# HanzhiC/TexPose

Hardware: AMD Instinct MI355X
Metric: rendered rays/sec (480x640x128 samples) + train iters/sec (higher is better)
Workload: dtype f32 carried as 2xf16 (f16x3 products, f32 accumulate); 1 GPU; Duck-like synthetic scene 480x640, 128 samples/ray, batch=1 image per GPU, forward render (render_by_slices mode='val', all pixels), per-sample outputs materialised; samples_per_ray=128, mlp_precision=f16x3, parallelism=images sharded across 1 GPU(s), no collective

## Files before the change

include/texpose_amd.h:

```cpp
#ifndef TEXPOSE_AMD_H
#define TEXPOSE_AMD_H

#include <stddef.h>
#include <stdint.h>

#ifdef __cplusplus
extern "C" {
#endif

typedef void* tp_stream_t;

#define TP_ABI_VERSION 16

int tp_abi_version(void);
const char* tp_last_error(void);

enum tp_pixel_mode {
  TP_PIX_COORDS = 0,
  TP_PIX_INDEX = 1
};
enum tp_bounds_mode {
  TP_BOUNDS_MAP = 0,
  TP_BOUNDS_AABB = 1,
  TP_BOUNDS_NONE = 2
// ... 96 lines not shown
  unsigned int* act_max;
  float* ray_bias;
  const float* density_noise;
} tp_mlp_fwd_args;
size_t tp_mlp_ray_bias_bytes(int B, int R);
enum { TP_MLP_FP32 = 0, TP_MLP_F16X3 = 1, TP_MLP_F16 = 2 };

int tp_mlp_fwd(const tp_mlp_fwd_args* args, tp_stream_t stream);

size_t tp_mlp_packed_t_bytes(void);
size_t tp_mlp_bwd_workspace_bytes(int64_t n_samples);
typedef struct tp_mlp_bwd_args {
  tp_mlp_weights weights;
  void* packed_t;
  int repack;
  const float* saved;
  const float* rgb; const float* density; const float* uncert;
  const float* g_rgb; const float* g_density; const float* g_uncert;
  const float* lat_trans;
  const float* lat_light;
  int B, R, N;
  float* g_rgb_w[4];   float* g_rgb_b[4];
  float* g_trans_w[4]; float* g_trans_b[4];
  float* g_lat_trans;
  float* g_lat_light;
  void* workspace;
  int wgrad_precision;
  int dz_max_is_clear;
  int wgrad_cus;
} tp_mlp_bwd_args;
int tp_mlp_bwd(const tp_mlp_bwd_args* args, tp_stream_t stream);

int tp_posenc(const float* x, int64_t n, int C, int L, float* out, tp_stream_t stream);

typedef struct tp_composite_args {
  const float* ray;
  const float* rgb;
  const float* density;
  const float* depth;
  const float* uncert;
  int64_t n; int N; float min_uncert;
  float* out_ray;
  float* alpha_static;
  float* alpha_transient;
  float* prob;
  float* rgb_ray;
  float* uncert_ray;
} tp_composite_args;
int tp_composite_fwd(const tp_composite_args* args, tp_stream_t stream);

typedef struct tp_composite_bwd_args {
  tp_composite_args fwd;
  const float* g_out_ray;
  const float* g_alpha_static;
  const float* g_alpha_transient;
  const float* g_prob;
  float* g_rgb;
  float* g_density;
  float* g_uncert;
  const float* g_rgb_ray;
  const float* g_uncert_ray;
  const float* g_rgb_ray2;
  const float* g_rgb_ray3;
  const float* g_density_add;
} tp_composite_bwd_args;
int tp_composite_bwd(const tp_composite_bwd_args* args, tp_stream_t stream);

typedef struct tp_render_eval_args {
  tp_raygen_args raygen;
  const void* packed;
  const float* lat_trans;
  const float* lat_light;
  int precision;
  int* status;
  float min_uncert;
  void* workspace;
  float* out_ray;
  float* alpha_static;
  float* alpha_transient;
  int packed_ray_bias;
} tp_render_eval_args;
size_t tp_render_eval_workspace_bytes(int B, int R, int N);
int tp_render_eval(const tp_render_eval_args* args, tp_stream_t stream);

typedef struct tp_patch_gather_args {
  const float* coords;
  const float* image;
  const float* image_syn;
  const float* nocs;
  const float* normal;
  const float* obj_mask;
  const float* mask_syn;
  int B, P, H, W;
  float* out;
  const float* disc_rgb; float* disc_real; float* disc_fake; int disc_geo; int pad_;
} tp_patch_gather_args;
int tp_patch_gather(const tp_patch_gather_args* args, tp_stream_t stream);

typedef struct tp_eval_metrics_args {
  const float* rgb_static;
  const float* image;
  const float* obj_mask;
  int B, h, w;
  int out_h, out_w;
  void* workspace;
  double* out;
} tp_eval_metrics_args;
int64_t tp_eval_metrics_workspace_bytes(int B, int out_h, int out_w);
int tp_eval_metrics(const tp_eval_metrics_args* args, tp_stream_t stream);

#define TP_SN_MAX_WEIGHTS 8
#define TP_SN_MAX_SLABS 8
#define TP_SN_MAX_SETS 3
typedef struct tp_sn_weight {
  const float* weight;
  float* u;
  float* v;
  float* weight_sn;
  float* sigma;
  const float* grad_sn;
  float* grad;
  float* work;
  int rows, cols;
  float* u_out;
  float* v_out;
  int32_t accumulate;
  const float* grad_sn2; const float* weight_sn2; const float* u2; const float* v2; const float* sigma2;
} tp_sn_weight;
int64_t tp_sn_work_floats(int rows, int cols);
int tp_sn_fwd(const tp_sn_weight* weights, int n, int training, tp_stream_t stream);
int tp_sn_fwd_sets(const tp_sn_weight* weights, int n, int n_sets, tp_stream_t stream);
int tp_sn_bwd(const tp_sn_weight* weights, int n, tp_stream_t stream);
typedef struct tp_sn_step_tail {
  const float* terms[4]; float weights[4]; int n_terms; int word_finite;
  float* total;
  int32_t* bad; int32_t* snapshot; int n_bad; int pad_;
  float* param[TP_SN_MAX_WEIGHTS];
  float* square_avg[TP_SN_MAX_WEIGHTS];
  float* step[TP_SN_MAX_WEIGHTS];
  const float* lr_dev; float lr_host, alpha, one_minus_alpha, eps;
} tp_sn_step_tail;
int tp_sn_bwd_step(const tp_sn_weight* weights, int n, const tp_sn_step_tail* tail, tp_stream_t stream);

#define TP_NERF_LOSSES_MAX_BLOCKS 1024
typedef struct tp_nerf_losses_args {
  const float* rgb;
  const float* uncert;
  const float* density;
  const float* gathered;
  int B, P, N;
  void* workspace;
  double* sums;
  float* losses;
  uint32_t* ticket;
} tp_nerf_losses_args;
int tp_nerf_losses_fwd(const tp_nerf_losses_args* args, tp_stream_t stream);
int tp_nerf_losses_bwd(const tp_nerf_losses_args* args, const float* g_render, const float* g_unc, const float* g_trans,
                       float* g_rgb, float* g_uncert, float* g_density, tp_stream_t stream);
int tp_nerf_losses_bwd_total(const tp_nerf_losses_args* args, const float* g_render, const float* g_unc, const float* g_trans,
                             float* g_rgb, float* g_uncert, float* g_density, const float* const* terms, const float* weights, int n,
                             float* out, const int32_t* mlp_status, int32_t* bad, int n_bad, int word_status, int word_finite,
                             int32_t* snapshot, uint64_t* step_counter, tp_stream_t stream);

int tp_inorm_lrelu_fwd(const float* x, int64_t n_inst, int hw, float eps, float slope, float* y, float* xhat, float* rstd,
                       tp_stream_t stream);
int tp_inorm_lrelu_bwd(const float* xhat, const float* rstd, const float* gy, int64_t n_inst, int hw, float slope,
// ... 542 lines not shown
```

texpose_amd/csrc/render_eval.hip:

```cpp
#include "tp_common.h"

namespace {
size_t align256(size_t x) { return (x + 255) / 256 * 256; }
struct Layout { size_t center, ray, depth, rgb, density, uncert, mlp_ws, ray_bias, total; };
Layout layout(int64_t B, int64_t R, int64_t N) {
  Layout l;
  size_t o = 0;
  l.center = o; o += align256((size_t)B * R * 3 * 4);
  l.ray = o;    o += align256((size_t)B * R * 3 * 4);
  l.depth = o;  o += align256((size_t)B * R * N * 4);
  l.rgb = o;    o += align256((size_t)B * R * N * 6 * 4);
  l.density = o; o += align256((size_t)B * R * N * 2 * 4);
  l.uncert = o; o += align256((size_t)B * R * N * 4);
  l.mlp_ws = o; o += align256(tp_mlp_workspace_bytes(B * R * N));
  l.ray_bias = o; o += align256(tp_mlp_ray_bias_bytes((int)B, (int)R));
  l.total = o;
  return l;
}
}

extern "C" size_t tp_render_eval_workspace_bytes(int B, int R, int N) { return layout(B, R, N).total; }

extern "C" int tp_render_eval(const tp_render_eval_args* a, tp_stream_t stream) {
  TP_REQUIRE(a && a->workspace && a->out_ray && a->packed && a->lat_trans && a->lat_light, "null pointer");
  TP_REQUIRE(a->raygen.B > 0 && a->raygen.R > 0 && a->raygen.N > 0, "bad sizes");
  const int B = a->raygen.B, R = a->raygen.R, N = a->raygen.N;
  const Layout l = layout(B, R, N);
  char* ws = (char*)a->workspace;
  tp_raygen_args rg = a->raygen;
  rg.center = (float*)(ws + l.center); rg.ray = (float*)(ws + l.ray); rg.depth = (float*)(ws + l.depth);
  rg.near = nullptr; rg.far = nullptr;
  if (int rc = tp_raygen(&rg, stream)) return rc;
  tp_mlp_fwd_args m = {};
  m.packed = a->packed;
  m.center = rg.center; m.ray = rg.ray; m.depth = rg.depth;
  m.lat_trans = a->lat_trans; m.lat_light = a->lat_light;
  m.B = B; m.R = R; m.N = N;
  m.rgb = (float*)(ws + l.rgb); m.density = (float*)(ws + l.density); m.uncert = (float*)(ws + l.uncert);
  m.saved = nullptr; m.workspace = ws + l.mlp_ws; m.precision = a->precision; m.status = a->status;
  if (a->packed_ray_bias) {
    TP_REQUIRE((a->precision == TP_MLP_F16X3 || a->precision == TP_MLP_F16) && N % 128 == 0,
               "tp_render_eval: packed_ray_bias needs TP_MLP_F16X3 or TP_MLP_F16 and N % 128 == 0");
    m.ray_bias = (float*)(ws + l.ray_bias);
  }
  if (int rc = tp_mlp_fwd(&m, stream)) return rc;
  tp_composite_args c = {};
  c.ray = rg.ray; c.rgb = m.rgb; c.density = m.density; c.depth = rg.depth; c.uncert = m.uncert;
  c.n = (int64_t)B * R; c.N = N; c.min_uncert = a->min_uncert;
  c.out_ray = a->out_ray; c.alpha_static = a->alpha_static; c.alpha_transient = a->alpha_transient; c.prob = nullptr;
  return tp_composite_fwd(&c, stream);
}
```

texpose_amd/graph.py:

```python
from __future__ import annotations

import itertools
import warnings

import torch
import torch.nn.functional as torch_F

from . import autograd_ops, knobs, ops
from .geometry import FlexPatchSampler, RaySampler, rotation_distance
from .nerf import NeRF
from .options import AttrDict as edict

RENDER_KEYS = ("rgb", "rgb_static", "rgb_transient", "opacity", "opacity_static", "opacity_transient", "uncert",
               "depth", "alpha_static", "alpha_transient", "density")

_philox_calls = itertools.count()
_ones_cache = {}


def _ones_like_cached(t):
    key = (tuple(t.shape), t.dtype, str(t.device))
    if key not in _ones_cache:
        _ones_cache[key] = torch.ones_like(t).detach()
    return _ones_cache[key]


class RenderMixin:

    HOST_REQUIRED = ("nerf", "lab_loss", "latent_vars_trans", "latent_vars_light", "MSE_loss", "compute_gan_loss")
    HOST_OPTIONAL = (
        "fuse_prologue",
        "step_counter",
        "range_fallbacks",
        "perceptual_loss",
        "feat_stream",
    )

    @staticmethod
    def _jitter(opt, rand, step_counter=None):
        if rand is not None:
            return dict(rand=rand)
        if opt.nerf.sample_stratified and step_counter is not None:
            return dict(jitter=ops.JITTER_PHILOX, seed=torch.initial_seed() & (2 ** 64 - 1), offset=0, offset_dev=step_counter)
        if opt.nerf.sample_stratified:
            return dict(jitter=ops.JITTER_PHILOX, seed=torch.initial_seed() & (2 ** 64 - 1), offset=next(_philox_calls))
        return dict(jitter=ops.JITTER_MID)

    @staticmethod
    def sample_depth(opt, batch_size, depth_range, num_rays=None, rand=None):
        near, far = depth_range
        return ops.sample_depth(near, far, opt.nerf.sample_intvs, depth_param=RenderMixin._depth_param(opt), **RenderMixin._jitter(opt, rand))[..., None]

    @staticmethod
    def _depth_param(opt):
        param = opt.nerf.depth.param
        if param not in ops.DEPTH_PARAMS:
            raise KeyError(param)
        return param

    @staticmethod
    def ray_batch_sample(ray_identity, ray_idx):
        assert ray_identity.shape[0] == ray_idx.shape[0]
        C = ray_identity.shape[-1]
        return torch.gather(ray_identity, 1, ray_idx[..., None].expand(-1, -1, C))

    def render(self, opt, pose, intr=None, ray_idx=None, depth_range=None, sample_idx=None, mode=None, rand=None):
        N = opt.nerf.sample_intvs
        z_near, z_far = depth_range
        batch_size = len(pose)
        src = dict(coords=ray_idx) if mode == "train" else dict(ray_idx=ray_idx)
        rows_k13 = (mode == "train" and torch.is_tensor(sample_idx) and sample_idx.dim() == 1 and sample_idx.is_cuda
                    and self.latent_vars_trans.weight.shape[0] == self.latent_vars_light.weight.shape[0])
        fused = {}
        if mode == "train" and getattr(self, "fuse_prologue", False):
            job = ray_idx.__dict__.pop("_tp_sampler_job", None)
            if job is not None:
                fused["sampler"] = job
            if rows_k13:
                lat_t, lat_l, fused["rows"] = autograd_ops.latent_rows(self.latent_vars_trans.weight, self.latent_vars_light.weight, sample_idx,
                                                                       defer=True)
        elif torch.is_tensor(ray_idx) and "_tp_sampler_job" in ray_idx.__dict__:
            raise RuntimeError("render: ray_idx comes from a deferred sampler call but this render does not fill it (fuse_prologue is off)")
        center, ray, _, _, depth = ops.raygen(intr, pose, H=opt.H, W=opt.W, n_samples=N, z_near=z_near, z_far=z_far,
                                              ndc=bool(opt.camera.ndc), depth_param=self._depth_param(opt), **src, **fused,
                                              **self._jitter(opt, rand, getattr(self, "step_counter", None) if mode == "train" else None))
        depth_samples = depth[..., None]
        if "rows" in fused:
            pass
        elif rows_k13:
            lat_t, lat_l = autograd_ops.latent_rows(self.latent_vars_trans.weight, self.latent_vars_light.weight, sample_idx)
        elif mode == "train" and torch.is_tensor(sample_idx) and sample_idx.dim() == 1:
            lat_t = self.latent_vars_trans.weight.index_select(0, sample_idx)
            lat_l = self.latent_vars_light.weight.index_select(0, sample_idx)
        elif mode == "train":
            lat_t = self.latent_vars_trans.weight[sample_idx]
            lat_l = self.latent_vars_light.weight[sample_idx]
        elif mode == "val":
            lat_t = self.latent_vars_trans.weight[0][None]
            lat_l = self.latent_vars_light.weight[0][None]
        else:
            if opt.render.transient == "zero":
                lat_t = torch.zeros(batch_size, opt.nerf.N_latent_trans, device=pose.device)
            elif opt.render.transient == "sample":
                lat_t = self.latent_vars_trans.weight[sample_idx][None]
            else:
                raise NotImplementedError
            lat_l = self.latent_vars_light.weight[sample_idx][None]
        rgb_s, density_s, uncert_s = self.nerf.forward_samples(opt, center=center, ray=ray, depth_samples=depth_samples,
                                                               latent_variable_trans=lat_t, latent_variable_light=lat_l,
                                                               mode=mode)
        per_sample = bool(opt.render.get("per_sample", True)) or torch.is_grad_enabled()
        fan = dict(fan_out={}) if mode == "train" else {}
        (rgb, rgb_static, rgb_transient, depth_map, opacity, opacity_static, opacity_transient, _prob, uncert,
         alpha_static, alpha_transient) = self.nerf.composite(opt, ray, rgb_s, density_s, depth_samples, uncert_s,
                                                              per_sample=per_sample, want_prob=False, **fan)
        ret = edict(rgb=rgb, rgb_static=rgb_static, rgb_transient=rgb_transient, opacity=opacity,
                    opacity_static=opacity_static, opacity_transient=opacity_transient, uncert=uncert,
                    depth=depth_map, alpha_static=alpha_static, alpha_transient=alpha_transient, density=density_s)
        ret.update(fan.get("fan_out") or {})
        return ret

    def _range_guarded(self, opt, device, render_image):
        out = render_image()
        nerf = self.nerf
        if not set(ops.F16_RANGE_PRECISIONS) & {nerf.precision, nerf.train_precision} or opt.arch.get("mlp_range_check", "sync") == "off" \
                or torch.cuda.is_current_stream_capturing():
            return out
        if ops.take_mlp_status(device) & 1:
            self.range_fallbacks = getattr(self, "range_fallbacks", 0) + 1
            if self.range_fallbacks == 1:
                warnings.warn("texpose_amd: an activation left the fp16 range of the f16x3 / f16 MLP kernel; the image was "
                              "re-rendered with the exact-fp32 kernel (arch.mlp_precision='fp32' avoids the double work)")
            keep = nerf.precision, nerf.train_precision
            nerf.precision = nerf.train_precision = "fp32"
            try:
                out = render_image()
            finally:
                nerf.precision, nerf.train_precision = keep
        return out

    @staticmethod
    def _slice_rays(opt):
        return int(opt.nerf.get("slice_rays") or max(opt.nerf.rand_rays, min(opt.H * opt.W, 1 << 20)))

    def render_by_slices(self, opt, pose, intr=None, depth_range=None, object_mask=None, sample_idx=None, mode=None):
        return self._range_guarded(opt, pose.device, lambda: self._render_by_slices(
            opt, pose, intr=intr, depth_range=depth_range, object_mask=object_mask, sample_idx=sample_idx, mode=mode))

    def _render_by_slices(self, opt, pose, intr=None, depth_range=None, object_mask=None, sample_idx=None, mode=None):
        HW = opt.H * opt.W
        step = self._slice_rays(opt)
        if mode == "val":
            parts = {k: [] for k in RENDER_KEYS}
            for c in range(0, HW, step):
                idx = torch.arange(c, min(c + step, HW), device=pose.device)[None]
                ret = self.render(opt, pose, intr=intr, ray_idx=idx, depth_range=depth_range, sample_idx=sample_idx,
                                  mode=mode)
                for k in RENDER_KEYS:
                    parts[k].append(ret[k])
            return edict({k: (None if v[0] is None else (v[0] if len(v) == 1 else torch.cat(v, dim=1))) for k, v in parts.items()})
        dev, N = pose.device, opt.nerf.sample_intvs
        obj = (object_mask.reshape(HW) > 0).nonzero(as_tuple=True)[0]
        out = edict()
        lazy = not bool(opt.render.get("per_sample", True))
        for k in RENDER_KEYS:
            if lazy and "alpha" in k:
                out[k] = None
            elif k == "uncert":
                out[k] = torch.full((1, HW, 1), float(opt.nerf.min_uncert), device=dev)
            elif k == "density":
                out[k] = torch.ones(1, HW, N, 2, device=dev)
            elif "rgb" in k:
                out[k] = torch.zeros(1, HW, 3, device=dev)
            elif "alpha" in k:
                out[k] = torch.ones(1, HW, N, device=dev)
            else:
                out[k] = torch.zeros(1, HW, 1, device=dev)
        for c in range(0, len(obj), step):
            idx = obj[c:c + step][None]
            ret = self.render(opt, pose, intr=intr, ray_idx=idx, depth_range=depth_range, sample_idx=sample_idx,
                              mode=mode)
            for k in RENDER_KEYS:
                if out[k] is not None:
                    out[k][:, idx[0]] = ret[k][0]
        return out

    def gather_patches(self, opt, var, disc_rgb=None):
        B = len(var.idx)
        if var.get("gathered_for") is var.ray_idx:
            return var
        args = (var.ray_idx, var.image, var.get("image_syn", var.image),
                var.get("nocs_pred", var.image), var.get("normal_pred", var.image),
                var.obj_mask.view(B, opt.H, opt.W), var.get("mask_syn", var.obj_mask).view(B, opt.H, opt.W))
        if disc_rgb is not None and disc_rgb.is_cuda and not knobs.K.no_gather_disc:
            g, real, fake = ops.patch_gather(*args, disc_rgb=disc_rgb, disc_geo=bool(opt.gan.geo_conditional))
            var.disc_stacks = (real, fake, disc_rgb)
        else:
            g = ops.patch_gather(*args)
        var.gathered, var.gathered_for = g, var.ray_idx
        var.image_sample, var.image_syn_sample = g[:, 0:3], g[:, 3:6]
        var.nocs_sample, var.normal_sample = g[:, 6:9], g[:, 9:12]
        var.mask_sample, var.mask_syn_sample = g[:, 12:13], g[:, 13:14]
        return var

    def sample_geometry(self, opt, var, mode=None):
        if mode == "train":
            if "nocs_sample" not in var:
                var = self.gather_patches(opt, var)
            return var
        B = len(var.idx)
        ms = (var.mask_syn > 0).float().view(B, 1, opt.H, opt.W)
        var.nocs_sample, var.normal_sample = var.nocs_pred * ms, var.normal_pred * ms
        return var

    def evaluate_metrics(self, opt, var, lpips_module=None):
        out_hw = None if list(opt.data.image_size) == [128, 128] else (480, 640)
        psnr, ssim, _ = ops.eval_metrics(var.rgb_static, var.image, var.obj_mask, opt.H, opt.W, out_hw=out_hw)
        out = edict(psnr=psnr, ssim=ssim)
        if lpips_module is not None:
            B = var.image.shape[0]
            rgb_map = var.rgb_static.view(B, opt.H, opt.W, 3).permute(0, 3, 1, 2)
            image, mask = var.image.view(B, 3, opt.H, opt.W), var.obj_mask.view(B, 1, opt.H, opt.W).float()
            if out_hw is not None:
                rgb_map = torch_F.interpolate(rgb_map, size=list(out_hw), mode="bilinear", align_corners=False)
                image = torch_F.interpolate(image, size=list(out_hw), mode="bilinear", align_corners=False)
                mask = torch_F.interpolate(mask, size=list(out_hw), mode="nearest")
            with torch.no_grad():
                out.lpips = lpips_module(rgb_map * 2 - 1, (image * mask) * 2 - 1).reshape(-1).mean()
        return out

    def _warn_once(self, message):
        seen = self.__dict__.setdefault("_warned", set())
        if message not in seen:
            seen.add(message)
            warnings.warn("texpose_amd: " + message)

    def _lab_loss_torch(self):
        if "_lab_module" not in self.__dict__:
            from .lab import LabLoss
            self.__dict__["_lab_module"] = LabLoss()
        return self.__dict__["_lab_module"]

    def compute_loss(self, opt, var, mode=None, train_step="nerf"):
        loss = edict()
        B = len(var.idx)
        patch_mode = bool(opt.nerf.rand_rays and mode in ["train", "test-optim"])
        if patch_mode:
            _, h, w, _ = var.ray_idx.shape
            var = self.gather_patches(opt, var)
            image, obj_mask = var.image_sample, var.mask_sample
            image_syn, mask_syn = var.image_syn_sample, var.mask_syn_sample
            rgb = var.rgb.view(B, h, w, 3).permute(0, 3, 1, 2)
            uncert = var.uncert.view(B, h, w, 1).permute(0, 3, 1, 2)
        else:
            image = var.image.view(B, 3, opt.H, opt.W)
            obj_mask = (var.obj_mask > 0).float().view(B, 1, opt.H, opt.W)
            image_syn = var.get("image_syn", var.image).view(B, 3, opt.H, opt.W)
            mask_syn = (var.get("mask_syn", var.obj_mask) > 0).float().view(B, 1, opt.H, opt.W)
            rgb = var.rgb.view(B, opt.H, opt.W, 3).permute(0, 3, 1, 2)
            uncert = var.uncert.view(B, opt.H, opt.W, 1).permute(0, 3, 1, 2)
            var.image_syn_sample, var.image_sample, var.mask_sample, var.mask_syn_sample = (image_syn, image, obj_mask,
                                                                                            mask_syn)
        lw = opt.loss_weight
        if train_step == "nerf":
            fused = ("gathered" in var and opt.nerf.mask_obj and lw.render is not None and lw.uncert is not None
                     and lw.trans_reg is not None and lw.mask is None and var.rgb.is_cuda)
            if fused:
                loss.render, loss.uncert, loss.trans_reg = autograd_ops.nerf_losses(var.rgb, var.uncert,
# ... 244 lines not shown
```

texpose_amd/ops/render.py:

```python
from typing import Dict, Optional, Tuple

import torch

from .. import _lib, knobs
from .._lib import (BOUNDS_AABB, BOUNDS_MAP, BOUNDS_NONE, CompositeArgs, CompositeBwdArgs, JITTER_GIVEN, JITTER_MID, MLP_F16, MLP_F16X3, MLP_FP32,
                    MlpBwdArgs, MlpFwdArgs, MlpWeights, PACK_ALL, PACK_F16, PACK_F16X3, PACK_HEADS, PACK_RAYBIAS, PACK_TRUNK, PIX_COORDS, PIX_INDEX,
                    PatchGatherArgs, RaygenArgs)
from ._base import Tensor, _call, _f32, _float3, _on_tensor_device, _ptr

__all__ = ["DEPTH_PARAMS", "PRECISIONS", "F16_RANGE_PRECISIONS", "INFERENCE_ONLY_PRECISIONS", "COMPOSITE_RAY_FIELDS", "raygen", "aabb_intersect",
           "sample_depth", "packed_bytes", "pack_weights", "packed_t_bytes", "pack_heads_train", "_workspaces", "_workspace", "_status_words",
           "RANGE_MESSAGE", "mlp_status", "_act_max_words", "_track_act_max", "track_activation_max", "take_activation_max", "_act_max_ptr",
           "take_mlp_status", "check_mlp_status", "_status_polls", "poll_mlp_status", "mlp_forward", "ray_bias_applies", "_bwd_scratch",
           "mlp_backward", "posenc", "_composite_args", "composite_fwd", "composite_bwd", "patch_gather", "eval_metrics", "render_eval", "_lattices",
           "patch_coords", "latent_rows_fwd", "latent_rows_bwd"]

DEPTH_PARAMS = {"metric": _lib.DEPTH_METRIC, "inverse": _lib.DEPTH_INVERSE}
PRECISIONS = {"fp32": MLP_FP32, "f16x3": MLP_F16X3, "f16": MLP_F16}
F16_RANGE_PRECISIONS = ("f16x3", "f16")
INFERENCE_ONLY_PRECISIONS = ("f16",)

COMPOSITE_RAY_FIELDS = (("rgb", 0, 3), ("rgb_static", 3, 6), ("rgb_transient", 6, 9), ("depth", 9, 10),
                        ("opacity", 10, 11), ("opacity_static", 11, 12), ("opacity_transient", 12, 13),
                        ("uncert", 13, 14))


@_on_tensor_device
def raygen(intr: Tensor, pose: Tensor, *, H: int, W: int, n_samples: int = 0, coords: Optional[Tensor] = None,
           ray_idx: Optional[Tensor] = None, z_near: Optional[Tensor] = None, z_far: Optional[Tensor] = None,
           aabb: Optional[Tuple[Tuple[float, float, float], Tuple[float, float, float]]] = None,
           bg_range: Tuple[float, float] = (0.0, 30.0), rand: Optional[Tensor] = None,
           jitter: int = JITTER_MID, seed: int = 0, offset: int = 0, valid_rect: Optional[Tensor] = None,
           offset_dev: Optional[Tensor] = None, ndc: bool = False, depth_param: str = "metric",
           sampler: Optional[dict] = None, rows: Optional[dict] = None):
    intr, pose = _f32(intr, "intr"), _f32(pose, "pose")
    B = pose.shape[0]
    a = RaygenArgs()
    if coords is not None:
        coords = _f32(coords, "coords")
        R = coords.numel() // (2 * B)
        a.pixel_mode, a.coords = PIX_COORDS, coords.data_ptr()
    else:
        ray_idx = ray_idx.to(torch.int64).contiguous()
        R = ray_idx.numel() // B
        a.pixel_mode, a.ray_idx = PIX_INDEX, ray_idx.data_ptr()
    dev = pose.device
    center = torch.empty(B, R, 3, device=dev)
    ray = torch.empty(B, R, 3, device=dev)
    near = far = depth = None
    if aabb is not None:
        a.bounds_mode = BOUNDS_AABB
        a.aabb_min, a.aabb_max = _float3(aabb[0]), _float3(aabb[1])
        a.bg_near, a.bg_far = float(bg_range[0]), float(bg_range[1])
        if valid_rect is not None:
            valid_rect = _f32(valid_rect, "valid_rect")
            assert valid_rect.shape == (B, 4)
            a.valid_rect = valid_rect.data_ptr()
    elif z_near is not None:
        z_near, z_far = _f32(z_near, "z_near"), _f32(z_far, "z_far")
        assert z_near.numel() == B * H * W and z_far.numel() == B * H * W
        a.bounds_mode, a.z_near, a.z_far = BOUNDS_MAP, z_near.data_ptr(), z_far.data_ptr()
    else:
        a.bounds_mode = BOUNDS_NONE
    if a.bounds_mode != BOUNDS_NONE:
        near = torch.empty(B, R, device=dev)
        far = torch.empty(B, R, device=dev)
        a.near, a.far = near.data_ptr(), far.data_ptr()
        if n_samples > 0:
            depth = torch.empty(B, R, n_samples, device=dev)
            a.depth = depth.data_ptr()
    if rand is not None:
        rand = _f32(rand, "rand")
        assert rand.numel() == B * R * n_samples
        jitter = JITTER_GIVEN
        a.rand = rand.data_ptr()
    a.jitter_mode, a.seed, a.offset = jitter, seed, offset
    a.ndc, a.depth_param = int(bool(ndc)), DEPTH_PARAMS[depth_param]
    if offset_dev is not None:
        if offset_dev.dtype != torch.int64 or offset_dev.numel() != 1 or offset_dev.device != dev:
            raise ValueError("raygen: offset_dev must be one int64 word on the device of the inputs")
        a.offset_dev = offset_dev.data_ptr()
    a.intr, a.pose = intr.data_ptr(), pose.data_ptr()
    a.B, a.R, a.H, a.W, a.N = B, R, H, W, n_samples
    a.center, a.ray = center.data_ptr(), ray.data_ptr()
    if sampler is None and rows is None:
        _call("tp_raygen", a)
        return center, ray, near, far, depth
    sj = rj = None
    if sampler is not None:
        if coords is None or coords.data_ptr() != sampler["coords"].data_ptr() or sampler["B"] != B:
            raise ValueError("raygen: a sampler job fills ITS coords tensor -- pass that tensor as coords")
        sj = _lib.PatchSamplerJob()
        lo = sampler["lo"]
        sj.u, sj.p, sj.lattice = _ptr(sampler["u"]), sampler["p"], sampler["lattice"].data_ptr()
        sj.lo_dev = lo.data_ptr() if torch.is_tensor(lo) else None
        sj.lo_host = 0.0 if torch.is_tensor(lo) else float(lo)
        sj.span_host, sj.hi = float(sampler["hi"]) - sj.lo_host, float(sampler["hi"])
# ... 356 lines not shown


@_on_tensor_device
def patch_gather(coords: Tensor, image: Tensor, image_syn: Tensor, nocs: Tensor, normal: Tensor, obj_mask: Tensor,
                 mask_syn: Tensor, disc_rgb: Optional[Tensor] = None, disc_geo: bool = False):
    coords = _f32(coords, "coords")
    B, ph, pw, _ = coords.shape
    ts = [_f32(t, "image") for t in (image, image_syn, nocs, normal, obj_mask, mask_syn)]
    H, W = ts[0].shape[-2:]
    out = torch.empty(B, 14, ph, pw, device=coords.device)
    a = PatchGatherArgs()
    a.coords = coords.data_ptr()
    a.image, a.image_syn, a.nocs, a.normal, a.obj_mask, a.mask_syn = [t.data_ptr() for t in ts]
    a.B, a.P, a.H, a.W, a.out = B, ph * pw, H, W, out.data_ptr()
    if disc_rgb is None:
        _call("tp_patch_gather", a)
        return out
    rgb = _f32(disc_rgb.detach(), "disc_rgb")
    if rgb.numel() != B * ph * pw * 3:
        raise ValueError("patch_gather: disc_rgb [B,P,3] expected")
    nc = 9 if disc_geo else 3
    real, fake = torch.empty(2 * B, nc, ph, pw, device=coords.device), torch.empty(B, nc, ph, pw, device=coords.device)
    a.disc_rgb, a.disc_real, a.disc_fake, a.disc_geo = rgb.data_ptr(), real.data_ptr(), fake.data_ptr(), int(bool(disc_geo))
    _call("tp_patch_gather", a)
    return out, real, fake


@_on_tensor_device
def eval_metrics(rgb_static: Tensor, image: Tensor, obj_mask: Tensor, H: int, W: int, out_hw=None):
    rgb_static, image, obj_mask = _f32(rgb_static, "rgb_static"), _f32(image, "image"), _f32(obj_mask, "obj_mask")
    B = image.shape[0]
    if rgb_static.numel() != B * H * W * 3 or image.shape[1:] != (3, H, W) or obj_mask.numel() != B * H * W:
        raise ValueError("eval_metrics: rgb_static [B,H*W,3], image [B,3,H,W], obj_mask [B,H,W] expected")
    oh, ow = (H, W) if out_hw is None else (int(out_hw[0]), int(out_hw[1]))
    ws = torch.empty(max(1, _lib.load().tp_eval_metrics_workspace_bytes(B, oh, ow) // 4), device=image.device)
    out = torch.empty(B, 2, dtype=torch.float64, device=image.device)
    a = _lib.EvalMetricsArgs()
    a.rgb_static, a.image, a.obj_mask = rgb_static.data_ptr(), image.data_ptr(), obj_mask.data_ptr()
    a.B, a.h, a.w, a.out_h, a.out_w = B, H, W, oh, ow
    a.workspace, a.out = ws.data_ptr(), out.data_ptr()
    _call("tp_eval_metrics", a)
    n = float(B * 3 * oh * ow)
    mse = out[:, 0].sum() / n
    return -10.0 * torch.log10(mse), out[:, 1].sum() / n, mse


@_on_tensor_device
def render_eval(packed: Tensor, intr: Tensor, pose: Tensor, ray_idx: Tensor, z_near: Tensor, z_far: Tensor, lat_trans: Tensor,
                lat_light: Tensor, *, H: int, W: int, n_samples: int, precision: str = "f16x3", min_uncert: float = 0.05,
                rand: Optional[Tensor] = None, with_alphas: bool = False, ray_bias: bool = False, ndc: bool = False,
                depth_param: str = "metric"):
    intr, pose = _f32(intr, "intr"), _f32(pose, "pose")
    z_near, z_far = _f32(z_near, "z_near"), _f32(z_far, "z_far")
    lat_trans, lat_light = _f32(lat_trans, "lat_trans"), _f32(lat_light, "lat_light")
    ray_idx = ray_idx.to(torch.int64).contiguous()
    B, R = ray_idx.shape
    dev = pose.device
    a = _lib.RenderEvalArgs()
    rg = a.raygen
    rg.intr, rg.pose, rg.ray_idx, rg.z_near, rg.z_far = intr.data_ptr(), pose.data_ptr(), ray_idx.data_ptr(), z_near.data_ptr(), z_far.data_ptr()
    rg.B, rg.R, rg.H, rg.W, rg.N = B, R, H, W, n_samples
    rg.pixel_mode, rg.bounds_mode = PIX_INDEX, BOUNDS_MAP
    rg.ndc, rg.depth_param = int(bool(ndc)), DEPTH_PARAMS[depth_param]
    if rand is not None:
        rand = _f32(rand, "rand")
        rg.rand, rg.jitter_mode = rand.data_ptr(), JITTER_GIVEN
    else:
        rg.jitter_mode = JITTER_MID
    a.packed, a.lat_trans, a.lat_light = packed.data_ptr(), lat_trans.data_ptr(), lat_light.data_ptr()
    a.precision, a.min_uncert = PRECISIONS[precision], float(min_uncert)
    a.packed_ray_bias = 1 if ray_bias else 0
    a.status = mlp_status(dev).data_ptr() if precision in F16_RANGE_PRECISIONS else None
    ws = torch.empty(int(_lib.load().tp_render_eval_workspace_bytes(B, R, n_samples)) // 4 + 64, device=dev)
    out = torch.empty(B, R, 14, device=dev)
    a.workspace, a.out_ray = ws.data_ptr(), out.data_ptr()
    alphas = None
    if with_alphas:
        alphas = (torch.empty(B, R, n_samples, device=dev), torch.empty(B, R, n_samples, device=dev))
        a.alpha_static, a.alpha_transient = alphas[0].data_ptr(), alphas[1].data_ptr()
    _call("tp_render_eval", a)
    return (out, alphas) if with_alphas else out


_lattices = {}


@_on_tensor_device
def patch_coords(u: Optional[Tensor], patch_size: int, lo, hi: float, random_scale: bool = True, random_shift: bool = True, *,
                 nbatch: Optional[int] = None, seed: int = 0, counter: Optional[Tensor] = None, device=None, defer: bool = False):
    if u is not None:
        u = _f32(u, "u")
        B, dev = u.numel() // 3, u.device
    else:
        B, dev = int(nbatch), (counter.device if counter is not None else torch.device(device))
        if counter is not None and (counter.dtype != torch.int64 or counter.numel() != 1):
            raise ValueError("patch_coords: counter must be one int64 device word")
    p = int(patch_size)
    key = (p, dev.index)
    if key not in _lattices:
        _lattices[key] = torch.linspace(-1, 1, p, device=dev)
    coords = torch.empty(B, p, p, 2, device=dev)
    scales = torch.empty(B, 1, 1, 1, device=dev)
    if defer:
        coords._tp_sampler_job = dict(u=u, B=B, p=p, lattice=_lattices[key], lo=lo, hi=hi, random_scale=random_scale, random_shift=random_shift,
                                      seed=seed, counter=counter, coords=coords, scales=scales)
        return coords, scales
    lo_dev = lo.data_ptr() if torch.is_tensor(lo) else None
    lo_host = 0.0 if torch.is_tensor(lo) else float(lo)
    _call("tp_patch_coords", _ptr(u), B, p, _lattices[key].data_ptr(), lo_dev, lo_host, float(hi) - lo_host, float(hi), int(bool(random_scale)),
          int(bool(random_shift)), int(seed) & (2 ** 64 - 1), _ptr(counter), coords.data_ptr(), scales.data_ptr())
    return coords, scales


@_on_tensor_device
def latent_rows_fwd(w_trans: Tensor, w_light: Tensor, idx: Tensor, idx_copy: Optional[Tensor] = None, defer: bool = False):
    w_trans, w_light = _f32(w_trans, "w_trans"), _f32(w_light, "w_light")
    idx = idx.to(torch.int64).contiguous()
    B = idx.numel()
    ot, ol = torch.empty(B, w_trans.shape[1], device=idx.device), torch.empty(B, w_light.shape[1], device=idx.device)
    if idx_copy is not None and not (idx_copy.dtype == torch.int64 and idx_copy.is_contiguous() and idx_copy.numel() == B and idx_copy.device == idx.device):
        raise _lib.TexposeLibraryError("latent_rows_fwd: idx_copy must be a contiguous int64 device tensor of idx's length")
    if defer:
        return ot, ol, dict(w_trans=w_trans, w_light=w_light, idx=idx, out_trans=ot, out_light=ol, idx_copy=idx_copy)
    _call("tp_latent_rows_fwd", w_trans.data_ptr(), w_light.data_ptr(), idx.data_ptr(), B, w_trans.shape[1], w_light.shape[1], ot.data_ptr(),
          ol.data_ptr(), _ptr(idx_copy))
    return ot, ol


@_on_tensor_device
def latent_rows_bwd(g_trans: Tensor, g_light: Tensor, idx: Tensor, n_rows: int):
    g_trans, g_light = _f32(g_trans, "g_trans"), _f32(g_light, "g_light")
    if idx.dtype != torch.int64 or not idx.is_contiguous() or not idx.is_cuda:
        raise _lib.TexposeLibraryError("latent_rows_bwd: idx must be the contiguous int64 device tensor the forward used (got %s%s)"
                                       % (idx.dtype, "" if idx.is_contiguous() else ", non-contiguous"))
    B = idx.numel()
    gwt, gwl = torch.empty(n_rows, g_trans.shape[1], device=idx.device), torch.empty(n_rows, g_light.shape[1], device=idx.device)
    _call("tp_latent_rows_bwd", g_trans.data_ptr(), g_light.data_ptr(), idx.data_ptr(), B, int(n_rows), g_trans.shape[1], g_light.shape[1],
          gwt.data_ptr(), gwl.data_ptr())
    return gwt, gwl
```

Baseline: 2.078 million rays/s.

## Fuse masked eval render with GPU mask compaction and scatter into full-image maps

Adds a fused evaluation path for single-image rendering. A two-pass GPU scan compacts the object mask into ray indices and per-pixel slots. A native call then runs raygen, MLP and composite on each slice of masked rays and scatters per-ray and per-sample outputs into full-image maps, writing default values for background pixels. This replaces the Python path of nonzero, a per-slice render and indexed assignment into each output, cutting host overhead and separate scatter kernels. It adds a host sync to read the masked-ray count and a new code path that must match the fallback's defaults.

```diff
diff --git a/include/texpose_amd.h b/include/texpose_amd.h
--- a/include/texpose_amd.h
+++ b/include/texpose_amd.h
@@ -202,6 +202,37 @@
 } tp_render_eval_args;
 size_t tp_render_eval_workspace_bytes(int B, int R, int N);
 int tp_render_eval(const tp_render_eval_args* args, tp_stream_t stream);
+
+size_t tp_mask_compact_workspace_bytes(int64_t HW);
+int tp_mask_compact(const float* mask, int64_t HW, int64_t* ray_idx, int32_t* slot, int32_t* count, int32_t* count_host,
+                    void* workspace, tp_stream_t stream);
+
+typedef struct tp_eval_scatter_args {
+  const int32_t* slot;
+  int64_t HW;
+  int N;
+  int slot0, count;
+  int fill_defaults;
+  float min_uncert;
+  int pad_;
+  const float* out_ray;
+  const float* density;
+  const float* alpha_static;
+  const float* alpha_transient;
+  float* rgb; float* rgb_static; float* rgb_transient;
+  float* depth; float* opacity; float* opacity_static; float* opacity_transient; float* uncert;
+  float* density_map;
+  float* alpha_static_map;
+  float* alpha_transient_map;
+} tp_eval_scatter_args;
+int tp_eval_scatter(const tp_eval_scatter_args* args, tp_stream_t stream);
+
+typedef struct tp_render_eval_masked_args {
+  tp_render_eval_args render;
+  tp_eval_scatter_args scatter;
+} tp_render_eval_masked_args;
+size_t tp_render_eval_masked_workspace_bytes(int R, int N);
+int tp_render_eval_masked(const tp_render_eval_masked_args* args, tp_stream_t stream);
 
 typedef struct tp_patch_gather_args {
   const float* coords;
diff --git a/texpose_amd/csrc/eval_scatter.hip b/texpose_amd/csrc/eval_scatter.hip
--- /dev/null
+++ b/texpose_amd/csrc/eval_scatter.hip
@@ -0,0 +1,210 @@
+#include "tp_common.h"
+
+namespace {
+
+constexpr int kCompactThreads = 256, kCompactPer = 8, kCompactBlock = kCompactThreads * kCompactPer;
+
+__device__ __forceinline__ int wave_incl_scan_i32(int v, int lane) {
+#pragma unroll
+  for (int d = 1; d < 64; d <<= 1) {
+    const int t = __shfl_up(v, d);
+    if (lane >= d) v += t;
+  }
+  return v;
+}
+
+__device__ __forceinline__ int block_excl_scan(int v, int& total) {
+  __shared__ int wave_sum[kCompactThreads / 64];
+  const int lane = threadIdx.x & 63, wave = threadIdx.x >> 6;
+  const int incl = wave_incl_scan_i32(v, lane);
+  __syncthreads();
+  if (lane == 63) wave_sum[wave] = incl;
+  __syncthreads();
+  int before = 0, all = 0;
+#pragma unroll
+  for (int w = 0; w < kCompactThreads / 64; ++w) {
+    const int s = wave_sum[w];
+    before += w < wave ? s : 0;
+    all += s;
+  }
+  total = all;
+  return before + incl - v;
+}
+
+__device__ __forceinline__ int flags_of(const float* mask, int64_t base, int64_t HW) {
+  int f = 0;
+#pragma unroll
+  for (int j = 0; j < kCompactPer; ++j) {
+    const int64_t i = base + j;
+    if (i < HW && mask[i] > 0.f) f |= 1 << j;
+  }
+  return f;
+}
+
+__global__ __launch_bounds__(kCompactThreads) void mask_count_kernel(const float* __restrict__ mask, int64_t HW, int* __restrict__ block_count) {
+  const int64_t base = (int64_t)blockIdx.x * kCompactBlock + (int64_t)threadIdx.x * kCompactPer;
+  int total;
+  block_excl_scan(__popc(flags_of(mask, base, HW)), total);
+  if (threadIdx.x == 0) block_count[blockIdx.x] = total;
+}
+
+__global__ __launch_bounds__(kCompactThreads) void mask_write_kernel(const float* __restrict__ mask, int64_t HW, const int* __restrict__ block_count,
+                                                                     int64_t* __restrict__ ray_idx, int* __restrict__ slot, int* __restrict__ count) {
+  int mine = 0;
+  for (int b = threadIdx.x; b < (int)blockIdx.x; b += kCompactThreads) mine += block_count[b];
+  int before;
+  block_excl_scan(mine, before);
+  const int64_t base = (int64_t)blockIdx.x * kCompactBlock + (int64_t)threadIdx.x * kCompactPer;
+  const int f = flags_of(mask, base, HW);
+  int total;
+  int at = before + block_excl_scan(__popc(f), total);
+#pragma unroll
+  for (int j = 0; j < kCompactPer; ++j) {
+    const int64_t i = base + j;
+    if (i >= HW) break;
+    const bool on = (f >> j) & 1;
+    slot[i] = on ? at : -1;
+    if (on) ray_idx[at++] = i;
+  }
+  if (blockIdx.x == gridDim.x - 1 && threadIdx.x == 0) *count = before + total;
+}
+
+typedef float v4f __attribute__((ext_vector_type(4)));
+
+template <int V> struct Vec;
+template <> struct Vec<4> { using type = v4f; };
+template <> struct Vec<1> { using type = float; };
+
+template <int V>
+__device__ __forceinline__ void scatter_unit(const tp_eval_scatter_args& a, uint32_t u, uint32_t units_per_pixel, const float* __restrict__ src,
+                                             float* __restrict__ dst) {
+  using T = typename Vec<V>::type;
+  const uint32_t p = u / units_per_pixel, r = u - p * units_per_pixel;
+  const int s = a.slot[p];
+  const uint32_t row = (uint32_t)(s - a.slot0);
+  T v;
+  if (s >= 0 && row < (uint32_t)a.count) v = ((const T*)src)[(size_t)row * units_per_pixel + r];
+  else if (s < 0 && a.fill_defaults) v = (T)(1.f);
+  else return;
+  __builtin_nontemporal_store(v, (T*)dst + u);
+}
+
+template <int V>
+__device__ __forceinline__ void scatter_rays(const tp_eval_scatter_args& a, int64_t group) {
+  const int64_t p0 = group * 4;
+  float v[4][14];
+  bool write[4];
+  bool all = p0 + 3 < a.HW;
+#pragma unroll
+  for (int k = 0; k < 4; ++k) {
+    const int64_t p = p0 + k;
+    const int s = p < a.HW ? a.slot[p] : 0x7fffffff;
+    const uint32_t row = (uint32_t)(s - a.slot0);
+    const bool mine = s >= 0 && row < (uint32_t)a.count;
+    write[k] = p < a.HW && (mine || (s < 0 && a.fill_defaults));
+    all = all && write[k];
+#pragma unroll
+    for (int j = 0; j < 14; ++j) v[k][j] = mine ? a.out_ray[(size_t)row * 14 + j] : (j == 13 ? a.min_uncert : 0.f);
+  }
+  float* const rgb3[3] = {a.rgb, a.rgb_static, a.rgb_transient};
+  float* const one[5] = {a.depth, a.opacity, a.opacity_static, a.opacity_transient, a.uncert};
+  if (V == 4 && all) {
+#pragma unroll
+    for (int m = 0; m < 3; ++m) {
+      v4f* d = (v4f*)(rgb3[m] + p0 * 3);
+      const int c = 3 * m;
+      d[0] = v4f{v[0][c], v[0][c + 1], v[0][c + 2], v[1][c]};
+      d[1] = v4f{v[1][c + 1], v[1][c + 2], v[2][c], v[2][c + 1]};
+      d[2] = v4f{v[2][c + 2], v[3][c], v[3][c + 1], v[3][c + 2]};
+    }
+#pragma unroll
+    for (int m = 0; m < 5; ++m) *(v4f*)(one[m] + p0) = v4f{v[0][9 + m], v[1][9 + m], v[2][9 + m], v[3][9 + m]};
+    return;
+  }
+#pragma unroll
+  for (int k = 0; k < 4; ++k) {
+    if (!write[k]) continue;
+    const int64_t p = p0 + k;
+#pragma unroll
+    for (int m = 0; m < 3; ++m) {
+#pragma unroll
+      for (int c = 0; c < 3; ++c) rgb3[m][p * 3 + c] = v[k][3 * m + c];
+    }
+#pragma unroll
+    for (int m = 0; m < 5; ++m) one[m][p] = v[k][9 + m];
+  }
+}
+
+template <int V>
+__global__ __launch_bounds__(256) void eval_scatter_kernel(tp_eval_scatter_args a, uint32_t ray_groups, uint32_t alpha_units, uint32_t density_units) {
+  const uint64_t total = (uint64_t)ray_groups + density_units + 2ull * alpha_units;
+  const uint32_t upp = (uint32_t)a.N / V;
+  for (uint64_t w = (uint64_t)blockIdx.x * blockDim.x + threadIdx.x; w < total; w += (uint64_t)gridDim.x * blockDim.x) {
+    if (w < ray_groups) {
+      scatter_rays<V>(a, (int64_t)w);
+      continue;
+    }
+    uint64_t u = w - ray_groups;
+    if (u < density_units) {
+      scatter_unit<V>(a, (uint32_t)u, 2 * upp, a.density, a.density_map);
+      continue;
+    }
+    u -= density_units;
+    if (u < alpha_units) scatter_unit<V>(a, (uint32_t)u, upp, a.alpha_static, a.alpha_static_map);
+    else scatter_unit<V>(a, (uint32_t)(u - alpha_units), upp, a.alpha_transient, a.alpha_transient_map);
+  }
+}
+
+bool aligned16(const void* p) { return ((uintptr_t)p & 15) == 0; }
+
+}
+
+extern "C" size_t tp_mask_compact_workspace_bytes(int64_t HW) {
+  const int64_t blocks = HW > 0 ? (HW + kCompactBlock - 1) / kCompactBlock : 1;
+  return (size_t)blocks * sizeof(int);
+}
+
+extern "C" int tp_mask_compact(const float* mask, int64_t HW, int64_t* ray_idx, int32_t* slot, int32_t* count, int32_t* count_host,
+                               void* workspace, tp_stream_t stream) {
+  TP_REQUIRE(mask && ray_idx && slot && count && workspace, "null pointer");
+  TP_REQUIRE(HW > 0 && HW < (int64_t)1 << 31, "HW must lie in [1, 2^31)");
+  const int blocks = (int)((HW + kCompactBlock - 1) / kCompactBlock);
+  hipStream_t s = (hipStream_t)stream;
+  hipLaunchKernelGGL(mask_count_kernel, dim3(blocks), dim3(kCompactThreads), 0, s, mask, HW, (int*)workspace);
+  hipLaunchKernelGGL(mask_write_kernel, dim3(blocks), dim3(kCompactThreads), 0, s, mask, HW, (const int*)workspace, ray_idx, slot, count);
+  if (int rc = tp::check_launch("tp_mask_compact")) return rc;
+  if (count_host) {
+    const hipError_t e = hipMemcpyAsync(count_host, count, sizeof(int32_t), hipMemcpyDeviceToHost, s);
+    if (e != hipSuccess) {
+      tp::set_error("tp_mask_compact: copy of the count: %s", hipGetErrorString(e));
+      return (int)e;
+    }
+  }
+  return 0;
+}
+
+extern "C" int tp_eval_scatter(const tp_eval_scatter_args* a, tp_stream_t stream) {
+  TP_REQUIRE(a && a->slot && a->rgb && a->rgb_static && a->rgb_transient && a->depth && a->opacity && a->opacity_static &&
+                 a->opacity_transient && a->uncert, "null pointer");
+  TP_REQUIRE(a->HW > 0 && a->HW < (int64_t)1 << 31 && a->N > 0 && a->slot0 >= 0 && a->count >= 0, "bad sizes");
+  TP_REQUIRE(!a->alpha_static_map == !a->alpha_transient_map, "the two alpha maps come together");
+  TP_REQUIRE(a->count == 0 || (a->out_ray && (!a->density_map || a->density) && (!a->alpha_static_map || (a->alpha_static && a->alpha_transient))),
+             "a map is asked for without its compact source");
+  if (a->count == 0 && !a->fill_defaults) return 0;
+  const void* ptrs[] = {a->density, a->alpha_static, a->alpha_transient, a->rgb, a->rgb_static, a->rgb_transient, a->depth, a->opacity,
+                        a->opacity_static, a->opacity_transient, a->uncert, a->density_map, a->alpha_static_map, a->alpha_transient_map};
+  bool vec = a->N % 4 == 0;
+  for (const void* p : ptrs) vec = vec && aligned16(p);
+  const int V = vec ? 4 : 1;
+  const uint64_t alpha_units = a->alpha_static_map ? (uint64_t)a->HW * (a->N / V) : 0;
+  const uint64_t density_units = a->density_map ? (uint64_t)a->HW * (2 * a->N / V) : 0;
+  TP_REQUIRE(alpha_units < 1ull << 32 && density_units < 1ull << 32, "a per-sample map of more than 2^32 stores");
+  const uint32_t ray_groups = (uint32_t)((a->HW + 3) / 4);
+  const uint64_t total = ray_groups + density_units + 2 * alpha_units;
+  const uint64_t want = (total + 255) / 256;
+  const int blocks = (int)(want < 8192 ? want : 8192);
+  hipStream_t s = (hipStream_t)stream;
+  if (vec) hipLaunchKernelGGL(eval_scatter_kernel<4>, dim3(blocks), dim3(256), 0, s, *a, ray_groups, (uint32_t)alpha_units, (uint32_t)density_units);
+  else hipLaunchKernelGGL(eval_scatter_kernel<1>, dim3(blocks), dim3(256), 0, s, *a, ray_groups, (uint32_t)alpha_units, (uint32_t)density_units);
+  return tp::check_launch("tp_eval_scatter");
+}
diff --git a/texpose_amd/csrc/render_eval.hip b/texpose_amd/csrc/render_eval.hip
--- a/texpose_amd/csrc/render_eval.hip
+++ b/texpose_amd/csrc/render_eval.hip
@@ -50,3 +50,46 @@
   c.out_ray = a->out_ray; c.alpha_static = a->alpha_static; c.alpha_transient = a->alpha_transient; c.prob = nullptr;
   return tp_composite_fwd(&c, stream);
 }
+
+namespace {
+struct MaskedLayout { size_t out_ray, alpha_static, alpha_transient, render, total; };
+MaskedLayout masked_layout(int64_t R, int64_t N) {
+  MaskedLayout l;
+  size_t o = 0;
+  l.out_ray = o;         o += align256((size_t)R * 14 * 4);
+  l.alpha_static = o;    o += align256((size_t)R * N * 4);
+  l.alpha_transient = o; o += align256((size_t)R * N * 4);
+  l.render = o;          o += layout(1, R, N).total;
+  l.total = o;
+  return l;
+}
+}
+
+extern "C" size_t tp_render_eval_masked_workspace_bytes(int R, int N) { return masked_layout(R, N).total; }
+
+extern "C" int tp_render_eval_masked(const tp_render_eval_masked_args* a, tp_stream_t stream) {
+  TP_REQUIRE(a, "null pointer");
+  tp_eval_scatter_args sc = a->scatter;
+  sc.out_ray = sc.density = sc.alpha_static = sc.alpha_transient = nullptr;
+  if (sc.count == 0) return tp_eval_scatter(&sc, stream);
+  TP_REQUIRE(a->render.workspace, "null pointer");
+  TP_REQUIRE(a->render.raygen.B == 1 && a->render.raygen.R == sc.count && a->render.raygen.N == sc.N && a->render.raygen.N > 0,
+             "one image, raygen.R == scatter.count and raygen.N == scatter.N expected");
+  TP_REQUIRE(a->render.raygen.pixel_mode == TP_PIX_INDEX && a->render.raygen.ray_idx && (int64_t)a->render.raygen.H * a->render.raygen.W == sc.HW,
+             "the pixels come as raygen.ray_idx into the H x W == scatter.HW image");
+  const int R = sc.count, N = sc.N;
+  const MaskedLayout l = masked_layout(R, N);
+  char* ws = (char*)a->render.workspace;
+  const bool alphas = sc.alpha_static_map != nullptr;
+  tp_render_eval_args r = a->render;
+  r.workspace = ws + l.render;
+  r.out_ray = (float*)(ws + l.out_ray);
+  r.alpha_static = alphas ? (float*)(ws + l.alpha_static) : nullptr;
+  r.alpha_transient = alphas ? (float*)(ws + l.alpha_transient) : nullptr;
+  if (int rc = tp_render_eval(&r, stream)) return rc;
+  sc.out_ray = r.out_ray;
+  sc.density = (const float*)(ws + l.render + layout(1, R, N).density);
+  sc.alpha_static = r.alpha_static;
+  sc.alpha_transient = r.alpha_transient;
+  return tp_eval_scatter(&sc, stream);
+}
diff --git a/texpose_amd/graph.py b/texpose_amd/graph.py
--- a/texpose_amd/graph.py
+++ b/texpose_amd/graph.py
@@ -9,6 +9,7 @@
 from . import autograd_ops, knobs, ops
 from .geometry import FlexPatchSampler, RaySampler, rotation_distance
 from .nerf import NeRF
+from .ops import render as ops_render
 from .options import AttrDict as edict
 
 RENDER_KEYS = ("rgb", "rgb_static", "rgb_transient", "opacity", "opacity_static", "opacity_transient", "uncert",
@@ -120,6 +121,15 @@
         ret.update(fan.get("fan_out") or {})
         return ret
 
+    def _eval_latents(self, opt, batch_size, sample_idx, device):
+        if opt.render.transient == "zero":
+            lat_t = torch.zeros(batch_size, opt.nerf.N_latent_trans, device=device)
+        elif opt.render.transient == "sample":
+            lat_t = self.latent_vars_trans.weight[sample_idx][None]
+        else:
+            raise NotImplementedError
+        return lat_t, self.latent_vars_light.weight[sample_idx][None]
+
     def _range_guarded(self, opt, device, render_image):
         out = render_image()
         nerf = self.nerf
@@ -159,6 +169,8 @@
                 for k in RENDER_KEYS:
                     parts[k].append(ret[k])
             return edict({k: (None if v[0] is None else (v[0] if len(v) == 1 else torch.cat(v, dim=1))) for k, v in parts.items()})
+        if self._fused_eval_applies(opt, pose, intr, depth_range):
+            return self._render_eval_fused(opt, pose, intr, depth_range, object_mask, sample_idx)
         dev, N = pose.device, opt.nerf.sample_intvs
         obj = (object_mask.reshape(HW) > 0).nonzero(as_tuple=True)[0]
         out = edict()
@@ -184,6 +196,34 @@
                 if out[k] is not None:
                     out[k][:, idx[0]] = ret[k][0]
         return out
+
+    @staticmethod
+    def _fused_eval_applies(opt, pose, intr, depth_range):
+        if not bool(opt.render.get("fused_eval", True)) or not pose.is_cuda or len(pose) != 1 or torch.is_grad_enabled():
+            return False
+        if intr is None or depth_range is None or ops_render._track_act_max:
+            return False
+        return (ops.mlp_forward is ops_render.mlp_forward and ops.raygen is ops_render.raygen
+                and ops.composite_fwd is ops_render.composite_fwd)
+
+    def _render_eval_fused(self, opt, pose, intr, depth_range, object_mask, sample_idx):
+        HW, N, dev = opt.H * opt.W, opt.nerf.sample_intvs, pose.device
+        nerf = self.nerf
+        obj, slot, count = ops.mask_compact(object_mask.reshape(HW))
+        maps = ops.eval_maps(HW, N, bool(opt.render.get("per_sample", True)), dev)
+        precision = nerf.precision
+        ray_bias = ops.ray_bias_applies(precision, N, False, True)
+        packed = lat_t = lat_l = None
+        if count:
+            packed = nerf.packed_weights(precision, ray_bias=ray_bias)
+            lat_t, lat_l = self._eval_latents(opt, 1, sample_idx, dev)
+        step = self._slice_rays(opt)
+        for c in range(0, max(count, 1), step):
+            ops.render_eval_masked(packed, intr, pose, obj[c:c + step], slot, depth_range[0], depth_range[1], lat_t, lat_l, maps,
+                                   slot0=c, fill_defaults=c == 0, H=opt.H, W=opt.W, precision=precision,
+                                   min_uncert=opt.nerf.min_uncert, ray_bias=ray_bias, ndc=bool(opt.camera.ndc),
+                                   depth_param=self._depth_param(opt), **(self._jitter(opt, None) if count else {}))
+        return edict({k: maps[k] for k in RENDER_KEYS})
 
     def gather_patches(self, opt, var, disc_rgb=None):
         B = len(var.idx)
diff --git a/texpose_amd/ops/render.py b/texpose_amd/ops/render.py
--- a/texpose_amd/ops/render.py
+++ b/texpose_amd/ops/render.py
@@ -6,13 +6,14 @@
 from .._lib import (BOUNDS_AABB, BOUNDS_MAP, BOUNDS_NONE, CompositeArgs, CompositeBwdArgs, JITTER_GIVEN, JITTER_MID, MLP_F16, MLP_F16X3, MLP_FP32,
                     MlpBwdArgs, MlpFwdArgs, MlpWeights, PACK_ALL, PACK_F16, PACK_F16X3, PACK_HEADS, PACK_RAYBIAS, PACK_TRUNK, PIX_COORDS, PIX_INDEX,
                     PatchGatherArgs, RaygenArgs)
-from ._base import Tensor, _call, _f32, _float3, _on_tensor_device, _ptr
+from ._base import Tensor, _call, _f32, _float3, _on_tensor_device, _ptr, _want_gpu
 
 __all__ = ["DEPTH_PARAMS", "PRECISIONS", "F16_RANGE_PRECISIONS", "INFERENCE_ONLY_PRECISIONS", "COMPOSITE_RAY_FIELDS", "raygen", "aabb_intersect",
            "sample_depth", "packed_bytes", "pack_weights", "packed_t_bytes", "pack_heads_train", "_workspaces", "_workspace", "_status_words",
            "RANGE_MESSAGE", "mlp_status", "_act_max_words", "_track_act_max", "track_activation_max", "take_activation_max", "_act_max_ptr",
            "take_mlp_status", "check_mlp_status", "_status_polls", "poll_mlp_status", "mlp_forward", "ray_bias_applies", "_bwd_scratch",
-           "mlp_backward", "posenc", "_composite_args", "composite_fwd", "composite_bwd", "patch_gather", "eval_metrics", "render_eval", "_lattices",
+           "mlp_backward", "posenc", "_composite_args", "composite_fwd", "composite_bwd", "patch_gather", "eval_metrics", "render_eval", "mask_compact", "eval_maps", "eval_scatter",
+           "render_eval_masked", "_count_words", "_lattices",
            "patch_coords", "latent_rows_fwd", "latent_rows_bwd"]
 
 DEPTH_PARAMS = {"metric": _lib.DEPTH_METRIC, "inverse": _lib.DEPTH_INVERSE}
@@ -535,6 +536,117 @@
     return (out, alphas) if with_alphas else out
 
 
+_count_words: Dict[int, Tuple[Tensor, Tensor]] = {}
+
+
+@_on_tensor_device
+def mask_compact(mask: Tensor, read_count: bool = True):
+    mask = _f32(mask, "mask").reshape(-1)
+    HW, dev = mask.numel(), mask.device
+    key = dev.index or 0
+    if key not in _count_words:
+        _count_words[key] = (torch.zeros(1, dtype=torch.int32, device=dev), torch.zeros(1, dtype=torch.int32).pin_memory())
+    count, host = _count_words[key]
+    ray_idx = torch.empty(HW, dtype=torch.int64, device=dev)
+    slot = torch.empty(HW, dtype=torch.int32, device=dev)
+    ws = torch.empty(max(1, int(_lib.load().tp_mask_compact_workspace_bytes(HW)) // 4), dtype=torch.int32, device=dev)
+    _call("tp_mask_compact", mask.data_ptr(), HW, ray_idx.data_ptr(), slot.data_ptr(), count.data_ptr(), host.data_ptr() if read_count else None,
+          ws.data_ptr())
+    if not read_count:
+        return ray_idx, slot, count.clone()
+    torch.cuda.current_stream().synchronize()
+    n = int(host[0])
+    return ray_idx[:n], slot, n
+
+
+def eval_maps(HW: int, n_samples: int, per_sample: bool, device) -> Dict[str, Optional[Tensor]]:
+    e = lambda *shape: torch.empty(1, HW, *shape, device=device)
+    maps = {k: e(hi - lo) for k, lo, hi in COMPOSITE_RAY_FIELDS}
+    maps["density"] = e(n_samples, 2)
+    maps["alpha_static"] = e(n_samples) if per_sample else None
+    maps["alpha_transient"] = e(n_samples) if per_sample else None
+    return maps
+
+
+def _scatter_args(a, slot: Tensor, maps: Dict[str, Optional[Tensor]], slot0: int, count: int, fill_defaults: bool, min_uncert: float) -> int:
+    HW = slot.numel()
+    _want_gpu("eval_scatter", slot, "slot", torch.int32, (HW,))
+    N = maps["density"].shape[-2]
+    for k, lo, hi in COMPOSITE_RAY_FIELDS:
+        _want_gpu("eval_scatter", maps[k], k, torch.float32, (1, HW, hi - lo))
+    _want_gpu("eval_scatter", maps["density"], "density", torch.float32, (1, HW, N, 2))
+    for k in ("alpha_static", "alpha_transient"):
+        if maps[k] is not None:
+            _want_gpu("eval_scatter", maps[k], k, torch.float32, (1, HW, N))
+    a.slot, a.HW, a.N, a.slot0, a.count = slot.data_ptr(), HW, N, int(slot0), int(count)
+    a.fill_defaults, a.min_uncert = int(bool(fill_defaults)), float(min_uncert)
+    a.rgb, a.rgb_static, a.rgb_transient = maps["rgb"].data_ptr(), maps["rgb_static"].data_ptr(), maps["rgb_transient"].data_ptr()
+    a.depth, a.opacity, a.opacity_static = maps["depth"].data_ptr(), maps["opacity"].data_ptr(), maps["opacity_static"].data_ptr()
+    a.opacity_transient, a.uncert = maps["opacity_transient"].data_ptr(), maps["uncert"].data_ptr()
+    a.density_map, a.alpha_static_map, a.alpha_transient_map = maps["density"].data_ptr(), _ptr(maps["alpha_static"]), _ptr(maps["alpha_transient"])
+    return N
+
+
+@_on_tensor_device
+def eval_scatter(slot: Tensor, maps: Dict[str, Optional[Tensor]], *, slot0: int = 0, count: int = 0, fill_defaults: bool = True,
+                 min_uncert: float = 0.05, out_ray: Optional[Tensor] = None, density: Optional[Tensor] = None,
+                 alpha_static: Optional[Tensor] = None, alpha_transient: Optional[Tensor] = None) -> Dict[str, Optional[Tensor]]:
+    a = _lib.EvalScatterArgs()
+    N = _scatter_args(a, slot, maps, slot0, count, fill_defaults, min_uncert)
+    keep = []
+    if count:
+        srcs = dict(out_ray=(out_ray, 14), density=(density, 2 * N))
+        if maps["alpha_static"] is not None:
+            srcs.update(alpha_static=(alpha_static, N), alpha_transient=(alpha_transient, N))
+        for name, (t, width) in srcs.items():
+            if t is None or t.numel() != count * width:
+                raise ValueError("eval_scatter: %s must hold %d x %d values" % (name, count, width))
+            keep.append(_f32(t, name))
+            setattr(a, name, keep[-1].data_ptr())
+    _call("tp_eval_scatter", a)
+    return maps
+
+
+@_on_tensor_device
+def render_eval_masked(packed: Tensor, intr: Tensor, pose: Tensor, ray_idx: Tensor, slot: Tensor, z_near: Tensor, z_far: Tensor,
+                       lat_trans: Tensor, lat_light: Tensor, maps: Dict[str, Optional[Tensor]], *, slot0: int, fill_defaults: bool, H: int,
+                       W: int, precision: str = "f16x3", min_uncert: float = 0.05, rand: Optional[Tensor] = None, jitter: int = JITTER_MID,
+                       seed: int = 0, offset: int = 0, ray_bias: bool = False, ndc: bool = False, depth_param: str = "metric"):
+    dev = pose.device
+    R = ray_idx.numel()
+    a = _lib.RenderEvalMaskedArgs()
+    N = _scatter_args(a.scatter, slot, maps, slot0, R, fill_defaults, min_uncert)
+    if R == 0:
+        _call("tp_render_eval_masked", a)
+        return maps
+    intr, pose = _f32(intr, "intr"), _f32(pose, "pose")
+    z_near, z_far = _f32(z_near, "z_near"), _f32(z_far, "z_far")
+    lat_trans, lat_light = _f32(lat_trans, "lat_trans"), _f32(lat_light, "lat_light")
+    if pose.shape[0] != 1 or lat_trans.shape != (1, 16) or lat_light.shape != (1, 48) or z_near.numel() != H * W or z_far.numel() != H * W:
+        raise ValueError("render_eval_masked: one image expected (pose [1,3,4], latent rows [1,16] / [1,48], bounds [1,H*W])")
+    if ray_idx.dtype != torch.int64 or not ray_idx.is_contiguous():
+        ray_idx = ray_idx.to(torch.int64).contiguous()
+    r = a.render
+    rg = r.raygen
+    rg.intr, rg.pose, rg.ray_idx, rg.z_near, rg.z_far = intr.data_ptr(), pose.data_ptr(), ray_idx.data_ptr(), z_near.data_ptr(), z_far.data_ptr()
+    rg.B, rg.R, rg.H, rg.W, rg.N = 1, R, H, W, N
+    rg.pixel_mode, rg.bounds_mode = PIX_INDEX, BOUNDS_MAP
+    rg.ndc, rg.depth_param = int(bool(ndc)), DEPTH_PARAMS[depth_param]
+    if rand is not None:
+        rand = _f32(rand, "rand")
+        assert rand.numel() == R * N
+        rg.rand, jitter = rand.data_ptr(), JITTER_GIVEN
+    rg.jitter_mode, rg.seed, rg.offset = jitter, seed, offset
+    r.packed, r.lat_trans, r.lat_light = packed.data_ptr(), lat_trans.data_ptr(), lat_light.data_ptr()
+    r.precision, r.min_uncert = PRECISIONS[precision], float(min_uncert)
+    r.packed_ray_bias = 1 if ray_bias else 0
+    r.status = mlp_status(dev).data_ptr() if precision in F16_RANGE_PRECISIONS else None
+    ws = torch.empty(int(_lib.load().tp_render_eval_masked_workspace_bytes(R, N)) // 4 + 64, device=dev)
+    r.workspace = ws.data_ptr()
+    _call("tp_render_eval_masked", a)
+    return maps
+
+
 _lattices = {}
 
 
```

After: 2.068 million rays/s. About the same (-0.5%).
